# mgdesaix/WGSassign

Measured on AMD Instinct MI355X. Metric: EM SNP-updates/s (per-population update, n_call=100), higher is better.
Workload: dtype f64; 1 GPU; 1 GPU(s), SNP-sharded: synthetic Beagle 10000000 SNPs x 1000 ind, K=10, EM sweep; mode=exact, snps_per_gpu=10000000, gl_bytes_per_gpu=80000000000, comm_native_rccl=False, step=wgs_em_fit iteration (enqueued ahead of the host)

## Files before the change

wgsassign_amd/csrc/codes_kernels.hip:

```cpp
#include "common.h"

namespace {

typedef float f4 __attribute__((ext_vector_type(4)));
typedef const f4 __attribute__((address_space(1))) *gf4_ptr;
typedef uint32_t __attribute__((address_space(1))) *gu32_ptr;
typedef unsigned long long __attribute__((address_space(1))) *gu64_ptr;
typedef uint8_t __attribute__((address_space(1))) *gu8_ptr;

constexpr unsigned long long KEY_EMPTY = ~0ull;
constexpr int ENC_SLOTS = WGS_ENC_SLOTS;
constexpr int ENC_RMAX = 24;
constexpr int ENC_PD = ENC_SLOTS >= 2048 ? 2 : 1;
constexpr int ENC_UQ = ENC_SLOTS >= 2048 ? 4 : 2;

__device__ __forceinline__ unsigned hash32(unsigned g0, unsigned g1)
{
    const unsigned x = g0 ^ __builtin_rotateleft32(g1, 13);
    return __umul24(x, 0x9E3779u) ^ __builtin_rotateleft32(__umul24(x >> 8, 0x85EBCBu), 3);
}

struct EncodeArgs {
    float4 *const *base;
    const int32_t *npairs, *ncols;
    const SlabCodes *slabs;
    int32_t n_slabs;
    int64_t m, tiles;
    float2 *dict;
    uint8_t *ncls;
    int32_t drows, lrows;
    int32_t batch, batch_cap;
    int64_t unit_stride;
    uint8_t *sample;
    unsigned long long *stats;
    uint4 *wave_stats;
};

enum EncStat {
    ST_SUM_NCLS = 0,
    ST_RICH = 1,
    ST_CMAX = 2,
    ST_ROWS_BATCH = 3,
    ST_UNUSED = 4,
    ST_ROUNDS = 5,
    ST_BUFFERS = 6,
    ST_DIRECT = 7,
    ST_COUNT = 8
};

#ifdef WGS_ENC_STATS
__device__ unsigned long long g_enc_stats[8];
#define ENC_CLOCK(i) do { const unsigned long long now_ = clock64(); stat_[i] += now_ - mark_; mark_ = now_; } while (0)
#else
#define ENC_CLOCK(i) do { } while (0)
#endif

template <int SNPS, bool SAMPLE>
__global__ __launch_bounds__(64, ENC_SLOTS >= 2048 ? 2 : 4) void class_encode_kernel(EncodeArgs A)
{
#ifdef WGS_ENC_STATS
    unsigned long long stat_[4] = {0, 0, 0, 0}, mark_ = clock64();
#endif
    constexpr int COLS = 64 / SNPS, T = ENC_SLOTS / SNPS, NW = T / 64;
    constexpr unsigned TMASK = T - 1, HSHIFT = T == 64 ? 26 : (T == 128 ? 25 : 24);
    constexpr int NL = 4 * ENC_UQ;
    __shared__ unsigned long long keys[ENC_SLOTS];
    __shared__ __align__(16) uint8_t gid_of[ENC_SLOTS];
    __shared__ __align__(16) uint8_t slot_of[ENC_SLOTS];
    const int lane = threadIdx.x;
    const int s = lane & (SNPS - 1), col = lane / SNPS;
    const int64_t unit = (int64_t)blockIdx.x * A.unit_stride;
    const int64_t tile = unit / (64 / SNPS);
    const int sub = (int)(unit - tile * (64 / SNPS));
    if (tile >= A.tiles) return;
    const int ls = sub * SNPS + s;
    const int64_t snp = tile * 64 + ls;

#pragma unroll
    for (int i = 0; i < ENC_SLOTS / 64; ++i) keys[i * 64 + lane] = KEY_EMPTY;
    __builtin_amdgcn_fence(__ATOMIC_RELEASE, "wavefront");

    bool rich = false;
    unsigned n_rounds = 0, n_buffers = 0;
    int nid = 0;

    auto snp_or = [&](bool v) {
        int x = v ? 1 : 0;
#pragma unroll
        for (int d = SNPS; d < 64; d <<= 1) x |= __shfl_xor(x, d, 64);
        return x != 0;
    };
    auto snp_or64 = [&](unsigned long long v) {
        unsigned lo = (unsigned)v, hi = (unsigned)(v >> 32);
#pragma unroll
        for (int d = SNPS; d < 64; d <<= 1) {
            lo |= (unsigned)__shfl_xor((int)lo, d, 64);
            hi |= (unsigned)__shfl_xor((int)hi, d, 64);
        }
        return ((unsigned long long)hi << 32) | lo;
    };
    auto snp_scan = [&](int cnt, int &pre, int &tot) {
        pre = 0;
        tot = 0;
#pragma unroll
        for (int c = 0; c < COLS; ++c) {
            const int v = __shfl(cnt, c * SNPS + s, 64);
            if (c < col) pre += v;
            tot += v;
        }
    };
    auto wave_max = [&](int v) {
#pragma unroll
        for (int off = 32; off > 0; off >>= 1) v = max(v, __shfl_xor(v, off, 64));
        return v;
    };
    auto probe = [&](unsigned slot, unsigned long long key) { return atomicCAS(&keys[slot * SNPS + s], KEY_EMPTY, key); };
    auto set_bit = [&](unsigned long long (&m)[NW], unsigned id) {
#pragma unroll
        for (int w = 0; w < NW; ++w)
            if (NW == 1 || (id >> 6) == (unsigned)w) m[w] |= 1ull << (id & 63u);
    };
    auto bits_below = [&](const unsigned long long (&m)[NW], unsigned id) {
        int r = 0;
#pragma unroll
        for (int w = 0; w < NW; ++w) {
            const unsigned long long below = (id >> 6) > (unsigned)w ? ~0ull : ((id >> 6) == (unsigned)w ? (1ull << (id & 63u)) - 1ull : 0ull);
            r += __popcll(m[w] & below);
        }
        return r;
    };
    auto count_bits = [&](const unsigned long long (&m)[NW]) {
        int r = 0;
#pragma unroll
        for (int w = 0; w < NW; ++w) r += __popcll(m[w]);
        return r;
    };
    auto pop_lowest = [&](unsigned long long (&m)[NW]) {
        int pos = 0;
        bool done = false;
#pragma unroll
        for (int w = 0; w < NW; ++w) {
            if (!done && m[w]) {
                pos = 64 * w + __builtin_ctzll(m[w]);
                m[w] &= m[w] - 1ull;
                done = true;
            }
        }
        return pos;
    };

    ENC_CLOCK(0);
    for (int g = 0; g < A.n_slabs; ++g) {
        const int np = A.npairs[g], nc = A.ncols[g];
        const SlabCodes sc = A.slabs[g];
        const int nquads = sc.nquads;
        if (nquads == 0) continue;
        gf4_ptr src = (gf4_ptr)A.base[g] + tile * np * 64 + ls;
        gu32_ptr cw = (gu32_ptr)sc.codes + tile * nquads * 64 + ls;
        unsigned long long seen[NW];
#pragma unroll
        for (int w = 0; w < NW; ++w) seen[w] = 0ull;
        f4 nxt[ENC_PD][ENC_UQ][2];
        auto fetch = [&](int qb, f4 (&dst)[ENC_UQ][2]) {
#pragma unroll
            for (int u = 0; u < ENC_UQ; ++u) {
                const int q = qb + u * COLS + col;
                dst[u][0] = __builtin_nontemporal_load(src + (int64_t)min(2 * q, np - 1) * 64);
                dst[u][1] = __builtin_nontemporal_load(src + (int64_t)min(2 * q + 1, np - 1) * 64);
            }
        };
        constexpr int QSTEP = COLS * ENC_UQ;
#pragma unroll
        for (int d = 0; d < ENC_PD; ++d)
            if (d == 0 || d * QSTEP < nquads) fetch(d * QSTEP, nxt[d]);
        for (int qb = 0; qb < nquads; qb += QSTEP) {
            f4 v[ENC_UQ][2];
#pragma unroll
            for (int u = 0; u < ENC_UQ; ++u) v[u][0] = nxt[0][u][0], v[u][1] = nxt[0][u][1];
#pragma unroll
            for (int d = 0; d + 1 < ENC_PD; ++d)
#pragma unroll
                for (int u = 0; u < ENC_UQ; ++u) nxt[d][u][0] = nxt[d + 1][u][0], nxt[d][u][1] = nxt[d + 1][u][1];
            if (qb + ENC_PD * QSTEP < nquads) fetch(qb + ENC_PD * QSTEP, nxt[ENC_PD - 1]);
            unsigned long long key[NL], old[NL];
            unsigned slot[NL];
#pragma unroll
            for (int u = 0; u < ENC_UQ; ++u) {
#pragma unroll
                for (int h = 0; h < 4; ++h) {
                    const f4 vv = v[u][h >> 1];
                    const unsigned g0 = __float_as_uint((h & 1) ? vv.z : vv.x), g1 = __float_as_uint((h & 1) ? vv.w : vv.y);
                    key[4 * u + h] = ((unsigned long long)g1 << 32) | g0;
                    slot[4 * u + h] = hash32(g0, g1) >> HSHIFT;
                }
            }
            bool pend[NL], live[NL];
            const bool plain = 4 * (qb + COLS * ENC_UQ) <= nc && !__any(rich);
            if (plain) {
#pragma unroll
                for (int i = 0; i < NL; ++i) old[i] = probe(slot[i], key[i]);
#pragma unroll
                for (int i = 0; i < NL; ++i) {
                    live[i] = true;
                    pend[i] = old[i] != KEY_EMPTY && old[i] != key[i];
                }
            } else {
#pragma unroll
                for (int u = 0; u < ENC_UQ; ++u) {
                    const int q = qb + u * COLS + col;
#pragma unroll
                    for (int h = 0; h < 4; ++h) {
                        const int i = 4 * u + h;
                        live[i] = 4 * q + h < nc && !rich;
                        old[i] = key[i];
                        if (live[i]) old[i] = probe(slot[i], key[i]);
                    }
                }
#pragma unroll
                for (int i = 0; i < NL; ++i) pend[i] = live[i] && old[i] != KEY_EMPTY && old[i] != key[i];
            }
            bool any_pend = false;
#pragma unroll
            for (int i = 0; i < NL; ++i) any_pend = any_pend || pend[i];
            int rounds = 0;
            while (__any(any_pend)) {
                if (++rounds > ENC_RMAX) {
                    rich = rich || any_pend;
                    break;
                }
#pragma unroll
                for (int i = 0; i < NL; ++i) {
                    if (__any(pend[i])) {
                        if (pend[i]) {
                            slot[i] = (slot[i] + 1) & TMASK;
                            old[i] = probe(slot[i], key[i]);
                        }
                    }
                }
                any_pend = false;
#pragma unroll
                for (int i = 0; i < NL; ++i) {
                    pend[i] = pend[i] && old[i] != KEY_EMPTY && old[i] != key[i];
                    any_pend = any_pend || pend[i];
                }
            }
            n_rounds += (unsigned)rounds;
            ++n_buffers;
            int ins = 0;
#pragma unroll
            for (int i = 0; i < NL; ++i) ins += (live[i] && !pend[i] && old[i] == KEY_EMPTY) ? 1 : 0;
            if (__any(ins != 0)) {
                int pre, tot;
                snp_scan(ins, pre, tot);
                int id = nid + pre;
#pragma unroll
                for (int i = 0; i < NL; ++i) {
                    if (live[i] && !pend[i] && old[i] == KEY_EMPTY) {
                        gid_of[slot[i] * SNPS + s] = (uint8_t)min(id, 255);
                        if (id < T) slot_of[id * SNPS + s] = (uint8_t)slot[i];
                        ++id;
                    }
                }
                nid += tot;
                __builtin_amdgcn_fence(__ATOMIC_ACQ_REL, "wavefront");
            }
            unsigned cid[NL];
#pragma unroll
            for (int i = 0; i < NL; ++i) cid[i] = gid_of[slot[i] * SNPS + s];
            if (!plain) {
#pragma unroll
                for (int i = 0; i < NL; ++i) cid[i] = (live[i] && !pend[i]) ? cid[i] : 0u;
            }
#pragma unroll
            for (int i = 0; i < NL; ++i)
                if (plain || (live[i] && !pend[i])) set_bit(seen, cid[i] < (unsigned)T ? cid[i] : 0u);
            if (!SAMPLE) {
#pragma unroll
                for (int u = 0; u < ENC_UQ; ++u) {
                    const int q = qb + u * COLS + col;
                    if (plain || q < nquads) cw[(int64_t)q * 64] = cid[4 * u] | (cid[4 * u + 1] << 8) | (cid[4 * u + 2] << 16) | (cid[4 * u + 3] << 24);
                }
            }
        }
        ENC_CLOCK(1);
        if (nid > T || nid > 254) rich = true;
        rich = snp_or(rich);
#pragma unroll
        for (int w = 0; w < NW; ++w) seen[w] = snp_or64(seen[w]);
        const int nloc = count_bits(seen);
        if (SAMPLE) {
            if (col == 0) A.sample[((int64_t)blockIdx.x * (A.n_slabs + 1) + g) * SNPS + s] = (uint8_t)(snp < A.m ? (rich ? 255 : min(nloc, 254)) : 0);
        } else {
            const int wmax = wave_max(rich ? 255 : nloc);
            if (lane < SNPS / WGS_ENC_MIN_SNPS) ((gu8_ptr)sc.tile_rows)[tile * WGS_TILE_ROWS_BYTES + sub * (SNPS / WGS_ENC_MIN_SNPS) + lane] = (uint8_t)wmax;
            if (A.lrows > 0 && wmax <= A.lrows) {
                const int rows_w = wmax;
                gu64_ptr ld = (gu64_ptr)sc.ldict + (tile * A.lrows) * 64 + ls;
                unsigned long long walk[NW];
#pragma unroll
                for (int w = 0; w < NW; ++w) walk[w] = seen[w];
                for (int c = 0; c < col; ++c) (void)pop_lowest(walk);
                for (int r0 = col; r0 < rows_w; r0 += COLS) {
                    unsigned long long e = 0;
                    if (r0 < nloc) {
                        const int id = pop_lowest(walk);
                        e = keys[(unsigned)slot_of[id * SNPS + s] * SNPS + s];
                        for (int c = 1; c < COLS; ++c) (void)pop_lowest(walk);
                    }
                    ld[(int64_t)r0 * 64] = e;
                }
                gu32_ptr lw = (gu32_ptr)sc.lcodes + tile * nquads * 64 + ls;
                constexpr int PF = 8;
                for (int q0 = col; q0 < nquads; q0 += COLS * PF) {
                    uint32_t w[PF];
#pragma unroll
                    for (int u = 0; u < PF; ++u) w[u] = cw[(int64_t)min(q0 + u * COLS, nquads - 1) * 64];
#pragma unroll
                    for (int u = 0; u < PF; ++u) {
                        if (q0 + u * COLS < nquads) {
                            uint32_t o = 0;
#pragma unroll
                            for (int h = 0; h < 4; ++h) o |= (uint32_t)(bits_below(seen, (w[u] >> (8 * h)) & 255u) & 255) << (8 * h);
                            lw[(int64_t)(q0 + u * COLS) * 64] = o;
                        }
                    }
                }
            }
        }
    }

    __builtin_amdgcn_fence(__ATOMIC_ACQ_REL, "wavefront");
    ENC_CLOCK(2);
    const int ncls = nid;
    if (ncls > A.drows || ncls > 254 || ncls > T) rich = true;
    for (int r0 = col; r0 < min(ncls, T); r0 += COLS)
        if (keys[(unsigned)slot_of[r0 * SNPS + s] * SNPS + s] == KEY_EMPTY) rich = true;
    rich = snp_or(rich);
    if (SAMPLE) {
        if (col == 0) A.sample[((int64_t)blockIdx.x * (A.n_slabs + 1) + A.n_slabs) * SNPS + s] = (uint8_t)(snp < A.m ? (rich ? 255 : min(ncls, 254)) : 0);
        return;
    }
    int eff = rich ? 0 : ncls;
    auto group_sum = [&](int v) {
#pragma unroll
        for (int off = 1; off < 16; off <<= 1)
            if (off < A.batch && off < SNPS) v += __shfl_xor(v, off, 64);
        return v;
    };
    for (int it = 0; it < 16; ++it) {
        const int sum = group_sum(eff);
        if (!__any(sum > A.batch_cap)) break;
        int best = (eff << 8) | (63 - (lane & 15));
#pragma unroll
        for (int off = 1; off < 16; off <<= 1)
            if (off < A.batch && off < SNPS) best = max(best, __shfl_xor(best, off, 64));
        if (sum > A.batch_cap && (best & 255) == 63 - (lane & 15)) {
            eff = 0;
            rich = true;
        }
    }
    if (col == 0) ((gu8_ptr)A.ncls)[snp] = (uint8_t)eff;
    {
        const int mb = wave_max(group_sum(eff)), mc = wave_max(eff);
        unsigned long long tot = (unsigned long long)((col == 0 && snp < A.m) ? eff : 0), nrich = (col == 0 && snp < A.m && rich) ? 1ull : 0ull;
#pragma unroll
        for (int off = 32; off > 0; off >>= 1) {
            tot += __shfl_xor(tot, off, 64);
            nrich += __shfl_xor(nrich, off, 64);
        }
        if (lane == 0) {
            typedef unsigned u4 __attribute__((ext_vector_type(4)));
            typedef u4 __attribute__((address_space(1))) *gu4_ptr;
            gu4_ptr rec = (gu4_ptr)A.wave_stats + 2 * (int64_t)blockIdx.x;
            rec[0] = u4{(unsigned)tot, (unsigned)nrich, (unsigned)mc, (unsigned)mb};
            rec[1] = u4{n_rounds, n_buffers, 0u, 0u};
        }
    }
    const int wmax = min(wave_max(eff), A.drows);
    gu64_ptr dd = (gu64_ptr)A.dict + (tile * A.drows) * 64 + ls;
    for (int r0 = col; r0 < wmax; r0 += COLS)
        if (r0 < eff) dd[(int64_t)r0 * 64] = keys[(unsigned)slot_of[r0 * SNPS + s] * SNPS + s];
#ifdef WGS_ENC_STATS
    ENC_CLOCK(3);
    if (lane == 0 && (blockIdx.x & 63u) == 0u) {
#pragma unroll
        for (int i = 0; i < 4; ++i) atomicAdd(&g_enc_stats[i], stat_[i]);
        atomicAdd(&g_enc_stats[4], 1ull);
    }
#endif
}

__global__ __launch_bounds__(256) void sample_hist_kernel(const uint8_t *sample, int64_t units, int n_slabs, const int32_t *ncols, unsigned long long *hist)
{
    __shared__ unsigned int hg[256], hl[256];
    hg[threadIdx.x] = hl[threadIdx.x] = 0;
    __syncthreads();
    constexpr int W = WGS_ENC_MIN_SNPS;
    for (int64_t i = threadIdx.x; i < units * W; i += 256) {
        const uint8_t *row = sample + (i / W) * (n_slabs + 1) * W;
        const int x = (int)(i % W);
        const unsigned g = row[n_slabs * W + x];
        if (g == 0) continue;
        atomicAdd(&hg[g], 1u);
        for (int sl = 0; sl < n_slabs; ++sl)
            if (ncols[sl]) atomicAdd(&hl[row[sl * W + x]], 1u);
    }
    __syncthreads();
    hist[threadIdx.x] = hg[threadIdx.x];
    hist[256 + threadIdx.x] = hl[threadIdx.x];
}

__global__ __launch_bounds__(256) void encode_stats_kernel(const uint4 *wave_stats, int64_t units, const SlabCodes *slabs, int n_slabs, int64_t tiles,
                                                           unsigned lrows, unsigned long long *out)
{
    unsigned long long sum = 0, rich = 0, rounds = 0, buffers = 0, direct = 0;
    unsigned cmax = 0, rows = 0;
    const int64_t step = (int64_t)gridDim.x * 256;
    for (int64_t u = (int64_t)blockIdx.x * 256 + threadIdx.x; u < units; u += step) {
        const uint4 a = wave_stats[2 * u], b = wave_stats[2 * u + 1];
        sum += a.x, rich += a.y, cmax = max(cmax, a.z), rows = max(rows, a.w), rounds += b.x, buffers += b.y;
    }
    for (int g = 0; g < n_slabs; ++g) {
        if (slabs[g].nquads == 0) continue;
        const unsigned long long *tr = reinterpret_cast<const unsigned long long *>(slabs[g].tile_rows);
        for (int64_t t = (int64_t)blockIdx.x * 256 + threadIdx.x; t < tiles; t += step) {
            unsigned mx = 0;
#pragma unroll
            for (int x = 0; x < WGS_TILE_ROWS_BYTES / 8; ++x) {
                const unsigned long long w = tr[t * (WGS_TILE_ROWS_BYTES / 8) + x];
#pragma unroll
                for (int k = 0; k < 8; ++k) mx = max(mx, (unsigned)((w >> (8 * k)) & 255u));
            }
            direct += mx > lrows ? 1u : 0u;
        }
    }
#pragma unroll
    for (int off = 32; off > 0; off >>= 1) {
        sum += __shfl_xor(sum, off, 64), rich += __shfl_xor(rich, off, 64), rounds += __shfl_xor(rounds, off, 64);
        buffers += __shfl_xor(buffers, off, 64), direct += __shfl_xor(direct, off, 64);
        cmax = max(cmax, (unsigned)__shfl_xor((int)cmax, off, 64)), rows = max(rows, (unsigned)__shfl_xor((int)rows, off, 64));
    }
    if ((threadIdx.x & 63) == 0) {
        atomicAdd(out + ST_SUM_NCLS, sum);
        atomicAdd(out + ST_RICH, rich);
        atomicMax(out + ST_CMAX, (unsigned long long)cmax);
        atomicMax(out + ST_ROWS_BATCH, (unsigned long long)rows);
        atomicAdd(out + ST_ROUNDS, rounds);
        atomicAdd(out + ST_BUFFERS, buffers);
        atomicAdd(out + ST_DIRECT, direct);
    }
}

}

static EncodeArgs encode_args(wgs_beagle *b, wgs_codes *c, const int32_t *d_ncols, unsigned long long *d_stats)
{
    EncodeArgs A;
    A.base = b->d_base;
    A.npairs = b->d_npairs;
    A.ncols = d_ncols;
    A.slabs = c->d_slabs;
    A.n_slabs = b->n_groups;
    A.m = b->m;
    A.tiles = wgs_ntiles(b->m);
    A.dict = c->dict;
    A.ncls = c->ncls;
    A.drows = c->drows;
    A.lrows = c->lrows;
    A.batch = c->score_batch;
    A.batch_cap = WGS_BATCH_ROWS_CAP;
    A.unit_stride = 1;
    A.sample = nullptr;
    A.stats = d_stats;
    A.wave_stats = nullptr;
    return A;
}

static int encode_scratch(wgs_beagle *b, int32_t **d_ncols, unsigned long long **d_stats, size_t extra = 0)
{
    std::vector<int32_t> ncols(b->n_groups);
    for (int g = 0; g < b->n_groups; ++g) ncols[g] = b->slabs[g].ncols;
    void *ws = nullptr;
    const size_t stat_bytes = sizeof(unsigned long long) * ST_COUNT;
    if (wgs_ctx_workspace(b->ctx, stat_bytes + sizeof(int32_t) * (b->n_groups + 64) + extra, &ws)) return 1;
    *d_stats = reinterpret_cast<unsigned long long *>(ws);
    *d_ncols = reinterpret_cast<int32_t *>(reinterpret_cast<char *>(ws) + stat_bytes);
    HIP_TRY(hipMemsetAsync(*d_stats, 0, stat_bytes, b->ctx->stream));
    HIP_TRY(hipMemcpyAsync(*d_ncols, ncols.data(), sizeof(int32_t) * b->n_groups, hipMemcpyHostToDevice, b->ctx->stream));
    HIP_TRY(hipStreamSynchronize(b->ctx->stream));
    return 0;
}

int launch_class_sample(wgs_beagle *b, wgs_codes *c, int max_units, unsigned long long *hist_g, unsigned long long *hist_l, double *rounds_per_buffer)
{
    int32_t *d_ncols = nullptr;
    unsigned long long *d_stats = nullptr;
    const int64_t units = wgs_ntiles(b->m) * WGS_TILE_ROWS_BYTES;
    const int64_t stride = std::max<int64_t>(1, units / std::max(1, max_units));
    const int64_t grid = (units + stride - 1) / stride;
    const size_t sample_bytes = ((size_t)grid * (b->n_groups + 1) * WGS_ENC_MIN_SNPS + 7) / 8 * 8, hist_bytes = 512 * sizeof(unsigned long long);
    if (encode_scratch(b, &d_ncols, &d_stats, sample_bytes + hist_bytes + 8)) return 1;
    EncodeArgs A = encode_args(b, c, d_ncols, d_stats);
    A.drows = 254;
    A.lrows = 0;
    A.unit_stride = stride;
    A.sample = reinterpret_cast<uint8_t *>(d_ncols + b->n_groups + 64);
    unsigned long long *d_hist = reinterpret_cast<unsigned long long *>((reinterpret_cast<uintptr_t>(A.sample + sample_bytes) + 7) & ~(uintptr_t)7);
    hipLaunchKernelGGL((class_encode_kernel<WGS_ENC_MIN_SNPS, true>), dim3((unsigned)grid), dim3(64), 0, b->ctx->stream, A);
    HIP_TRY(hipGetLastError());
    hipLaunchKernelGGL(sample_hist_kernel, dim3(1), dim3(256), 0, b->ctx->stream, A.sample, grid, (int)b->n_groups, d_ncols, d_hist);
    HIP_TRY(hipGetLastError());
    unsigned long long *h = reinterpret_cast<unsigned long long *>(b->ctx->pinned);
    HIP_TRY(hipMemcpyAsync(h, d_hist, hist_bytes, hipMemcpyDeviceToHost, b->ctx->stream));
    HIP_TRY(hipStreamSynchronize(b->ctx->stream));
    for (int i = 0; i < 256; ++i) {
        hist_g[i] = h[i];
        hist_l[i] = h[256 + i];
    }
    if (rounds_per_buffer) *rounds_per_buffer = 0.0;
    return 0;
}

int launch_class_encode(wgs_beagle *b, wgs_codes *c)
{
    int32_t *d_ncols = nullptr;
    unsigned long long *d_stats = nullptr;
    if (encode_scratch(b, &d_ncols, &d_stats)) return 1;
    const int64_t tiles = wgs_ntiles(b->m);
    EncodeArgs A = encode_args(b, c, d_ncols, d_stats);
    const int64_t units = tiles * (64 / c->snps_per_wave);
    A.wave_stats = c->wave_stats;
    WGS_REQUIRE(units < (1ll << 31), "class encoder: %lld work units exceed one launch", (long long)units);
    HIP_TRY(hipEventRecord(b->ctx->enc_ev0, b->ctx->stream));
    if (c->snps_per_wave == WGS_ENC_SLOTS / 64) hipLaunchKernelGGL((class_encode_kernel<WGS_ENC_SLOTS / 64, false>), dim3((unsigned)units), dim3(64), 0, b->ctx->stream, A);
    else if (c->snps_per_wave == WGS_ENC_SLOTS / 128) hipLaunchKernelGGL((class_encode_kernel<WGS_ENC_SLOTS / 128, false>), dim3((unsigned)units), dim3(64), 0, b->ctx->stream, A);
    else hipLaunchKernelGGL((class_encode_kernel<WGS_ENC_SLOTS / 256, false>), dim3((unsigned)units), dim3(64), 0, b->ctx->stream, A);
    HIP_TRY(hipGetLastError());
    HIP_TRY(hipEventRecord(b->ctx->enc_ev1, b->ctx->stream));
    {
        const unsigned gx = (unsigned)std::max<int64_t>(1, std::min<int64_t>(512, (units + 255) / 256));
        hipLaunchKernelGGL(encode_stats_kernel, dim3(gx), dim3(256), 0, b->ctx->stream, c->wave_stats, units, c->d_slabs, (int)b->n_groups, tiles,
                           (unsigned)(c->lrows > 0 ? c->lrows : 255), d_stats);
        HIP_TRY(hipGetLastError());
    }
    unsigned long long *h = reinterpret_cast<unsigned long long *>(b->ctx->pinned);
    HIP_TRY(hipMemcpyAsync(h, d_stats, sizeof(unsigned long long) * 8, hipMemcpyDeviceToHost, b->ctx->stream));
    HIP_TRY(hipStreamSynchronize(b->ctx->stream));
#ifdef WGS_ENC_STATS
    {
        unsigned long long st[8] = {0}, zero[8] = {0};
        (void)hipMemcpyFromSymbol(st, HIP_SYMBOL(g_enc_stats), sizeof st);
        (void)hipMemcpyToSymbol(HIP_SYMBOL(g_enc_stats), zero, sizeof zero);
        const double w = st[4] ? (double)st[4] : 1.0;
        fprintf(stderr, "[encode stats] %llu wavefronts sampled; cycles per wavefront: before the slabs %.0f, the slabs' walks %.0f, the slabs' ends %.0f, the end %.0f\n",
                st[4], st[0] / w, st[1] / w, st[2] / w, st[3] / w);
    }
#endif
    float ev_ms = 0.0f;
    if (hipEventElapsedTime(&ev_ms, b->ctx->enc_ev0, b->ctx->enc_ev1) == hipSuccess) c->kernel_ms = ev_ms;
    c->sum_ncls = (double)h[ST_SUM_NCLS];
    c->rich_snps = (int64_t)h[ST_RICH];
    c->cmax = (int32_t)h[ST_CMAX];
    c->rows_batch = std::max<int32_t>(c->score_batch, (int32_t)h[ST_ROWS_BATCH]);
    c->probe_rounds = h[ST_BUFFERS] ? (double)h[ST_ROUNDS] / (double)h[ST_BUFFERS] : 0.0;
    int64_t slab_tiles = 0;
    for (int g = 0; g < b->n_groups; ++g) slab_tiles += c->slabs[g].nquads ? tiles : 0;
    c->local_direct_share = c->lrows > 0 && slab_tiles ? (double)h[ST_DIRECT] / (double)slab_tiles : 1.0;
    return 0;
}
```

Measured before the change: 7.728 billion SNP-updates/s.

## Restructure class encoder probe loop with ballots, 32-bit addressing and identity-code shortcut

Restructures the class-encode kernel's hash-probe inner loop into a templated walk_buffer. It specialises on plain versus tail buffers, with a half-width variant for short tails, uses wave ballots to track pending probes, and precomputes flat LDS indices. Global loads and stores move to 32-bit byte offsets from per-tile bases. A fast path skips the local-code remapping when local ids equal global ids. The intent is to cut ALU, addressing and branching cost in the one-time encoder, but the measured metric is EM-iteration throughput, which this kernel likely does not affect. It also adds an ncols limit check and a debug dump path.

```diff
diff --git a/wgsassign_amd/csrc/codes_kernels.hip b/wgsassign_amd/csrc/codes_kernels.hip
--- a/wgsassign_amd/csrc/codes_kernels.hip
+++ b/wgsassign_amd/csrc/codes_kernels.hip
@@ -1,3 +1,5 @@
+#include <type_traits>
+
 #include "common.h"
 
 namespace {
@@ -17,7 +19,9 @@
 __device__ __forceinline__ unsigned hash32(unsigned g0, unsigned g1)
 {
     const unsigned x = g0 ^ __builtin_rotateleft32(g1, 13);
-    return __umul24(x, 0x9E3779u) ^ __builtin_rotateleft32(__umul24(x >> 8, 0x85EBCBu), 3);
+    unsigned y;
+    asm("v_mul_u32_u24 %0, %1, %2" : "=v"(y) : "s"(0x85EBCBu), "v"(x >> 8));
+    return __umul24(x, 0x9E3779u) ^ __builtin_rotateleft32(y, 3);
 }
 
 struct EncodeArgs {
@@ -62,8 +66,7 @@
     unsigned long long stat_[4] = {0, 0, 0, 0}, mark_ = clock64();
 #endif
     constexpr int COLS = 64 / SNPS, T = ENC_SLOTS / SNPS, NW = T / 64;
-    constexpr unsigned TMASK = T - 1, HSHIFT = T == 64 ? 26 : (T == 128 ? 25 : 24);
-    constexpr int NL = 4 * ENC_UQ;
+    constexpr unsigned HSHIFT = T == 64 ? 26 : (T == 128 ? 25 : 24);
     __shared__ unsigned long long keys[ENC_SLOTS];
     __shared__ __align__(16) uint8_t gid_of[ENC_SLOTS];
     __shared__ __align__(16) uint8_t slot_of[ENC_SLOTS];
@@ -74,7 +77,6 @@
     const int sub = (int)(unit - tile * (64 / SNPS));
     if (tile >= A.tiles) return;
     const int ls = sub * SNPS + s;
-    const int64_t snp = tile * 64 + ls;
 
 #pragma unroll
     for (int i = 0; i < ENC_SLOTS / 64; ++i) keys[i * 64 + lane] = KEY_EMPTY;
@@ -114,11 +116,11 @@
         for (int off = 32; off > 0; off >>= 1) v = max(v, __shfl_xor(v, off, 64));
         return v;
     };
-    auto probe = [&](unsigned slot, unsigned long long key) { return atomicCAS(&keys[slot * SNPS + s], KEY_EMPTY, key); };
-    auto set_bit = [&](unsigned long long (&m)[NW], unsigned id) {
-#pragma unroll
-        for (int w = 0; w < NW; ++w)
-            if (NW == 1 || (id >> 6) == (unsigned)w) m[w] |= 1ull << (id & 63u);
+    auto probe = [&](unsigned at, unsigned long long key) { return atomicCAS(&keys[at], KEY_EMPTY, key); };
+    auto set_bit = [&](unsigned long long (&m)[NW], unsigned id, bool on) {
+        const unsigned long long bit = 1ull << (id & 63u);
+#pragma unroll
+        for (int w = 0; w < NW; ++w) m[w] |= (on & (NW == 1 || (id >> 6) == (unsigned)w)) ? bit : 0ull;
     };
     auto bits_below = [&](const unsigned long long (&m)[NW], unsigned id) {
         int r = 0;
@@ -147,6 +149,113 @@
             }
         }
         return pos;
+    };
+
+    auto walk_buffer = [&](auto plain_c, auto nu_c, const int qb, const f4 (&v)[ENC_UQ][2], const int nc, const int nquads, const uint32_t cw_at,
+                           gu8_ptr cw_tile, unsigned long long (&seen)[NW]) {
+        constexpr bool PLAIN = decltype(plain_c)::value;
+        constexpr int NU = decltype(nu_c)::value, NLB = 4 * NU;
+        unsigned long long key[NLB], old[NLB];
+        unsigned ki[NLB];
+        bool live[NLB];
+#pragma unroll
+        for (int u = 0; u < NU; ++u) {
+#pragma unroll
+            for (int h = 0; h < 4; ++h) {
+                const f4 vv = v[u][h >> 1];
+                const unsigned g0 = __float_as_uint((h & 1) ? vv.z : vv.x), g1 = __float_as_uint((h & 1) ? vv.w : vv.y);
+                key[4 * u + h] = ((unsigned long long)g1 << 32) | g0;
+                ki[4 * u + h] = (hash32(g0, g1) >> HSHIFT) * SNPS + s;
+                live[4 * u + h] = PLAIN || (4 * (qb + u * COLS + col) + h < nc && !rich);
+            }
+        }
+#pragma unroll
+        for (int i = 0; i < NLB; ++i) {
+            if (PLAIN) {
+                old[i] = probe(ki[i], key[i]);
+            } else {
+                old[i] = key[i];
+                if (live[i]) old[i] = probe(ki[i], key[i]);
+            }
+        }
+        unsigned long long pm[NLB], any_pend = 0ull, any_ins = 0ull;
+        auto pending = [&](int i) { return (old[i] != KEY_EMPTY) & (old[i] != key[i]); };
+        auto inserted = [&](int i) { return live[i] & (old[i] == KEY_EMPTY); };
+#pragma unroll
+        for (int i = 0; i < NLB; ++i) {
+            pm[i] = __builtin_amdgcn_ballot_w64(pending(i));
+            any_pend |= pm[i];
+            any_ins |= __builtin_amdgcn_ballot_w64(inserted(i));
+        }
+        int rounds = 0;
+        while (any_pend) {
+            if (++rounds > ENC_RMAX) {
+                bool p = false;
+#pragma unroll
+                for (int i = 0; i < NLB; ++i) p = p | pending(i);
+                rich = rich || p;
+                break;
+            }
+#pragma unroll
+            for (int i = 0; i < NLB; ++i) {
+                if (pm[i]) {
+                    if (pending(i)) {
+                        ki[i] = (ki[i] + SNPS) & (unsigned)(ENC_SLOTS - 1);
+                        old[i] = probe(ki[i], key[i]);
+                    }
+                }
+            }
+            any_pend = 0ull;
+#pragma unroll
+            for (int i = 0; i < NLB; ++i) {
+                if (pm[i]) {
+                    pm[i] = __builtin_amdgcn_ballot_w64(pending(i));
+                    any_ins |= __builtin_amdgcn_ballot_w64(inserted(i));
+                }
+                any_pend |= pm[i];
+            }
+        }
+        n_rounds += (unsigned)rounds;
+        ++n_buffers;
+        if (any_ins) {
+            int ins = 0;
+#pragma unroll
+            for (int i = 0; i < NLB; ++i) ins += inserted(i) ? 1 : 0;
+            if (__any(ins != 0)) {
+                int pre, tot;
+                snp_scan(ins, pre, tot);
+                int id = nid + pre;
+#pragma unroll
+                for (int i = 0; i < NLB; ++i) {
+                    if (inserted(i)) {
+                        gid_of[ki[i]] = (uint8_t)min(id, 255);
+                        if (id < T) slot_of[id * SNPS + s] = (uint8_t)(ki[i] / SNPS);
+                        ++id;
+                    }
+                }
+                nid += tot;
+                __builtin_amdgcn_fence(__ATOMIC_ACQ_REL, "wavefront");
+            }
+        }
+        unsigned cid[NLB];
+#pragma unroll
+        for (int i = 0; i < NLB; ++i) cid[i] = gid_of[ki[i]];
+#pragma unroll
+        for (int i = 0; i < NLB; ++i) {
+            bool ok = true;
+            if (!PLAIN) {
+                ok = live[i] & !pending(i);
+                cid[i] = ok ? cid[i] : 0u;
+            }
+            set_bit(seen, cid[i], ok);
+        }
+        if (!SAMPLE) {
+#pragma unroll
+            for (int u = 0; u < NU; ++u) {
+                const uint32_t word = cid[4 * u] | (cid[4 * u + 1] << 8) | (cid[4 * u + 2] << 16) | (cid[4 * u + 3] << 24);
+                if (PLAIN || qb + u * COLS + col < nquads) *(gu32_ptr)(cw_tile + (cw_at + (uint32_t)(u * COLS * 256))) = word;
+            }
+        }
     };
 
     ENC_CLOCK(0);
@@ -155,21 +264,38 @@
         const SlabCodes sc = A.slabs[g];
         const int nquads = sc.nquads;
         if (nquads == 0) continue;
-        gf4_ptr src = (gf4_ptr)A.base[g] + tile * np * 64 + ls;
-        gu32_ptr cw = (gu32_ptr)sc.codes + tile * nquads * 64 + ls;
+        typedef const char __attribute__((address_space(1))) *gc8_ptr;
+        gc8_ptr src_tile = (gc8_ptr)((gf4_ptr)A.base[g] + tile * np * 64);
+        gu8_ptr cw_tile = (gu8_ptr)((gu32_ptr)sc.codes + tile * nquads * 64);
+        const uint32_t ls16 = (uint32_t)ls * 16u, ls4 = (uint32_t)ls * 4u;
         unsigned long long seen[NW];
 #pragma unroll
         for (int w = 0; w < NW; ++w) seen[w] = 0ull;
         f4 nxt[ENC_PD][ENC_UQ][2];
+#pragma unroll
+        for (int d = 0; d < ENC_PD; ++d)
+#pragma unroll
+            for (int u = 0; u < ENC_UQ; ++u) nxt[d][u][0] = nxt[d][u][1] = f4{0.0f, 0.0f, 0.0f, 0.0f};
+        constexpr int QSTEP = COLS * ENC_UQ;
         auto fetch = [&](int qb, f4 (&dst)[ENC_UQ][2]) {
-#pragma unroll
-            for (int u = 0; u < ENC_UQ; ++u) {
-                const int q = qb + u * COLS + col;
-                dst[u][0] = __builtin_nontemporal_load(src + (int64_t)min(2 * q, np - 1) * 64);
-                dst[u][1] = __builtin_nontemporal_load(src + (int64_t)min(2 * q + 1, np - 1) * 64);
+            if (2 * (qb + QSTEP) <= np) {
+                const uint32_t at = (uint32_t)(qb + col) * 2048u + ls16;
+#pragma unroll
+                for (int u = 0; u < ENC_UQ; ++u) {
+                    dst[u][0] = __builtin_nontemporal_load((gf4_ptr)(src_tile + (at + (uint32_t)(u * COLS * 2048))));
+                    dst[u][1] = __builtin_nontemporal_load((gf4_ptr)(src_tile + (at + (uint32_t)(u * COLS * 2048 + 1024))));
+                }
+            } else {
+#pragma unroll
+                for (int u = 0; u < ENC_UQ; ++u) {
+                    if (qb + u * COLS < nquads) {
+                        const int q = qb + u * COLS + col;
+                        dst[u][0] = __builtin_nontemporal_load((gf4_ptr)(src_tile + ((uint32_t)min(2 * q, np - 1) * 1024u + ls16)));
+                        dst[u][1] = __builtin_nontemporal_load((gf4_ptr)(src_tile + ((uint32_t)min(2 * q + 1, np - 1) * 1024u + ls16)));
+                    }
+                }
             }
         };
-        constexpr int QSTEP = COLS * ENC_UQ;
 #pragma unroll
         for (int d = 0; d < ENC_PD; ++d)
             if (d == 0 || d * QSTEP < nquads) fetch(d * QSTEP, nxt[d]);
@@ -182,105 +308,11 @@
 #pragma unroll
                 for (int u = 0; u < ENC_UQ; ++u) nxt[d][u][0] = nxt[d + 1][u][0], nxt[d][u][1] = nxt[d + 1][u][1];
             if (qb + ENC_PD * QSTEP < nquads) fetch(qb + ENC_PD * QSTEP, nxt[ENC_PD - 1]);
-            unsigned long long key[NL], old[NL];
-            unsigned slot[NL];
-#pragma unroll
-            for (int u = 0; u < ENC_UQ; ++u) {
-#pragma unroll
-                for (int h = 0; h < 4; ++h) {
-                    const f4 vv = v[u][h >> 1];
-                    const unsigned g0 = __float_as_uint((h & 1) ? vv.z : vv.x), g1 = __float_as_uint((h & 1) ? vv.w : vv.y);
-                    key[4 * u + h] = ((unsigned long long)g1 << 32) | g0;
-                    slot[4 * u + h] = hash32(g0, g1) >> HSHIFT;
-                }
-            }
-            bool pend[NL], live[NL];
-            const bool plain = 4 * (qb + COLS * ENC_UQ) <= nc && !__any(rich);
-            if (plain) {
-#pragma unroll
-                for (int i = 0; i < NL; ++i) old[i] = probe(slot[i], key[i]);
-#pragma unroll
-                for (int i = 0; i < NL; ++i) {
-                    live[i] = true;
-                    pend[i] = old[i] != KEY_EMPTY && old[i] != key[i];
-                }
-            } else {
-#pragma unroll
-                for (int u = 0; u < ENC_UQ; ++u) {
-                    const int q = qb + u * COLS + col;
-#pragma unroll
-                    for (int h = 0; h < 4; ++h) {
-                        const int i = 4 * u + h;
-                        live[i] = 4 * q + h < nc && !rich;
-                        old[i] = key[i];
-                        if (live[i]) old[i] = probe(slot[i], key[i]);
-                    }
-                }
-#pragma unroll
-                for (int i = 0; i < NL; ++i) pend[i] = live[i] && old[i] != KEY_EMPTY && old[i] != key[i];
-            }
-            bool any_pend = false;
-#pragma unroll
-            for (int i = 0; i < NL; ++i) any_pend = any_pend || pend[i];
-            int rounds = 0;
-            while (__any(any_pend)) {
-                if (++rounds > ENC_RMAX) {
-                    rich = rich || any_pend;
-                    break;
-                }
-#pragma unroll
-                for (int i = 0; i < NL; ++i) {
-                    if (__any(pend[i])) {
-                        if (pend[i]) {
-                            slot[i] = (slot[i] + 1) & TMASK;
-                            old[i] = probe(slot[i], key[i]);
-                        }
-                    }
-                }
-                any_pend = false;
-#pragma unroll
-                for (int i = 0; i < NL; ++i) {
-                    pend[i] = pend[i] && old[i] != KEY_EMPTY && old[i] != key[i];
-                    any_pend = any_pend || pend[i];
-                }
-            }
-            n_rounds += (unsigned)rounds;
-            ++n_buffers;
-            int ins = 0;
-#pragma unroll
-            for (int i = 0; i < NL; ++i) ins += (live[i] && !pend[i] && old[i] == KEY_EMPTY) ? 1 : 0;
-            if (__any(ins != 0)) {
-                int pre, tot;
-                snp_scan(ins, pre, tot);
-                int id = nid + pre;
-#pragma unroll
-                for (int i = 0; i < NL; ++i) {
-                    if (live[i] && !pend[i] && old[i] == KEY_EMPTY) {
-                        gid_of[slot[i] * SNPS + s] = (uint8_t)min(id, 255);
-                        if (id < T) slot_of[id * SNPS + s] = (uint8_t)slot[i];
-                        ++id;
-                    }
-                }
-                nid += tot;
-                __builtin_amdgcn_fence(__ATOMIC_ACQ_REL, "wavefront");
-            }
-            unsigned cid[NL];
-#pragma unroll
-            for (int i = 0; i < NL; ++i) cid[i] = gid_of[slot[i] * SNPS + s];
-            if (!plain) {
-#pragma unroll
-                for (int i = 0; i < NL; ++i) cid[i] = (live[i] && !pend[i]) ? cid[i] : 0u;
-            }
-#pragma unroll
-            for (int i = 0; i < NL; ++i)
-                if (plain || (live[i] && !pend[i])) set_bit(seen, cid[i] < (unsigned)T ? cid[i] : 0u);
-            if (!SAMPLE) {
-#pragma unroll
-                for (int u = 0; u < ENC_UQ; ++u) {
-                    const int q = qb + u * COLS + col;
-                    if (plain || q < nquads) cw[(int64_t)q * 64] = cid[4 * u] | (cid[4 * u + 1] << 8) | (cid[4 * u + 2] << 16) | (cid[4 * u + 3] << 24);
-                }
-            }
+            const uint32_t cw_at = (uint32_t)(qb + col) * 256u + ls4;
+            const bool plain = 4 * (qb + QSTEP) <= nc && !__any(rich);
+            if (plain) walk_buffer(std::true_type(), std::integral_constant<int, ENC_UQ>(), qb, v, nc, nquads, cw_at, cw_tile, seen);
+            else if (qb + (ENC_UQ / 2) * COLS >= nquads) walk_buffer(std::false_type(), std::integral_constant<int, ENC_UQ / 2>(), qb, v, nc, nquads, cw_at, cw_tile, seen);
+            else walk_buffer(std::false_type(), std::integral_constant<int, ENC_UQ>(), qb, v, nc, nquads, cw_at, cw_tile, seen);
         }
         ENC_CLOCK(1);
         if (nid > T || nid > 254) rich = true;
@@ -289,39 +321,49 @@
         for (int w = 0; w < NW; ++w) seen[w] = snp_or64(seen[w]);
         const int nloc = count_bits(seen);
         if (SAMPLE) {
-            if (col == 0) A.sample[((int64_t)blockIdx.x * (A.n_slabs + 1) + g) * SNPS + s] = (uint8_t)(snp < A.m ? (rich ? 255 : min(nloc, 254)) : 0);
+            if (col == 0) A.sample[((int64_t)blockIdx.x * (A.n_slabs + 1) + g) * SNPS + s] = (uint8_t)(tile * 64 + ls < A.m ? (rich ? 255 : min(nloc, 254)) : 0);
         } else {
             const int wmax = wave_max(rich ? 255 : nloc);
             if (lane < SNPS / WGS_ENC_MIN_SNPS) ((gu8_ptr)sc.tile_rows)[tile * WGS_TILE_ROWS_BYTES + sub * (SNPS / WGS_ENC_MIN_SNPS) + lane] = (uint8_t)wmax;
             if (A.lrows > 0 && wmax <= A.lrows) {
                 const int rows_w = wmax;
-                gu64_ptr ld = (gu64_ptr)sc.ldict + (tile * A.lrows) * 64 + ls;
+                const bool same_numbers = __all(bits_below(seen, (unsigned)nloc) == nloc);
+                gu8_ptr ld_tile = (gu8_ptr)((gu64_ptr)sc.ldict + (tile * A.lrows) * 64);
+                const uint32_t ls8 = (uint32_t)ls * 8u;
                 unsigned long long walk[NW];
 #pragma unroll
                 for (int w = 0; w < NW; ++w) walk[w] = seen[w];
-                for (int c = 0; c < col; ++c) (void)pop_lowest(walk);
+                if (!same_numbers)
+                    for (int c = 0; c < col; ++c) (void)pop_lowest(walk);
                 for (int r0 = col; r0 < rows_w; r0 += COLS) {
                     unsigned long long e = 0;
                     if (r0 < nloc) {
-                        const int id = pop_lowest(walk);
+                        int id = r0;
+                        if (!same_numbers) {
+                            id = pop_lowest(walk);
+                            for (int c = 1; c < COLS; ++c) (void)pop_lowest(walk);
+                        }
                         e = keys[(unsigned)slot_of[id * SNPS + s] * SNPS + s];
-                        for (int c = 1; c < COLS; ++c) (void)pop_lowest(walk);
                     }
-                    ld[(int64_t)r0 * 64] = e;
+                    *(gu64_ptr)(ld_tile + ((uint32_t)r0 * 512u + ls8)) = e;
                 }
-                gu32_ptr lw = (gu32_ptr)sc.lcodes + tile * nquads * 64 + ls;
-                constexpr int PF = 8;
-                for (int q0 = col; q0 < nquads; q0 += COLS * PF) {
+                gu8_ptr lw_tile = (gu8_ptr)((gu32_ptr)sc.lcodes + tile * nquads * 64);
+                constexpr int PF = COLS >= 16 ? 2 : 4;
+                for (int q0 = 0; q0 < nquads; q0 += COLS * PF) {
                     uint32_t w[PF];
 #pragma unroll
-                    for (int u = 0; u < PF; ++u) w[u] = cw[(int64_t)min(q0 + u * COLS, nquads - 1) * 64];
+                    for (int u = 0; u < PF; ++u)
+                        if (q0 + u * COLS < nquads) w[u] = *(gu32_ptr)(cw_tile + ((uint32_t)min(q0 + u * COLS + col, nquads - 1) * 256u + ls4));
 #pragma unroll
                     for (int u = 0; u < PF; ++u) {
                         if (q0 + u * COLS < nquads) {
-                            uint32_t o = 0;
-#pragma unroll
-                            for (int h = 0; h < 4; ++h) o |= (uint32_t)(bits_below(seen, (w[u] >> (8 * h)) & 255u) & 255) << (8 * h);
-                            lw[(int64_t)(q0 + u * COLS) * 64] = o;
+                            uint32_t o = w[u];
+                            if (!same_numbers) {
+                                o = 0;
+#pragma unroll
+                                for (int h = 0; h < 4; ++h) o |= (uint32_t)(bits_below(seen, (w[u] >> (8 * h)) & 255u) & 255) << (8 * h);
+                            }
+                            if (q0 + u * COLS + col < nquads) *(gu32_ptr)(lw_tile + ((uint32_t)(q0 + u * COLS + col) * 256u + ls4)) = o;
                         }
                     }
                 }
@@ -331,6 +373,7 @@
 
     __builtin_amdgcn_fence(__ATOMIC_ACQ_REL, "wavefront");
     ENC_CLOCK(2);
+    const int64_t snp = tile * 64 + ls;
     const int ncls = nid;
     if (ncls > A.drows || ncls > 254 || ncls > T) rich = true;
     for (int r0 = col; r0 < min(ncls, T); r0 += COLS)
@@ -531,6 +574,14 @@
     const int64_t units = tiles * (64 / c->snps_per_wave);
     A.wave_stats = c->wave_stats;
     WGS_REQUIRE(units < (1ll << 31), "class encoder: %lld work units exceed one launch", (long long)units);
+    for (int g = 0; g < b->n_groups; ++g)
+        WGS_REQUIRE((int64_t)b->slabs[g].ncols < (1ll << 22), "class encoder: a slab of %lld individuals exceeds its addressing", (long long)b->slabs[g].ncols);
+#ifdef WGS_ENC_DUMP
+    {
+        const size_t head = ((sizeof(SlabCodes) * b->n_groups + 255) / 256) * 256;
+        if (b->pool_bytes > head) HIP_TRY(hipMemsetAsync(reinterpret_cast<char *>(b->pool) + head, 0, b->pool_bytes - head, b->ctx->stream));
+    }
+#endif
     HIP_TRY(hipEventRecord(b->ctx->enc_ev0, b->ctx->stream));
     if (c->snps_per_wave == WGS_ENC_SLOTS / 64) hipLaunchKernelGGL((class_encode_kernel<WGS_ENC_SLOTS / 64, false>), dim3((unsigned)units), dim3(64), 0, b->ctx->stream, A);
     else if (c->snps_per_wave == WGS_ENC_SLOTS / 128) hipLaunchKernelGGL((class_encode_kernel<WGS_ENC_SLOTS / 128, false>), dim3((unsigned)units), dim3(64), 0, b->ctx->stream, A);
@@ -546,6 +597,36 @@
     unsigned long long *h = reinterpret_cast<unsigned long long *>(b->ctx->pinned);
     HIP_TRY(hipMemcpyAsync(h, d_stats, sizeof(unsigned long long) * 8, hipMemcpyDeviceToHost, b->ctx->stream));
     HIP_TRY(hipStreamSynchronize(b->ctx->stream));
+#ifdef WGS_ENC_DUMP
+    {
+        auto digest = [&](const char *name, int g, const void *dev, size_t bytes) {
+            std::vector<unsigned long long> host((bytes + 7) / 8, 0ull);
+            if (bytes && hipMemcpy(host.data(), dev, bytes, hipMemcpyDeviceToHost) != hipSuccess) return;
+            unsigned long long a = 0x9E3779B97F4A7C15ull, x = 0ull;
+            for (size_t i = 0; i < host.size(); ++i) {
+                a = (a ^ host[i]) * 0x100000001B3ull;
+                a ^= a >> 29;
+                x += host[i] * (2 * (unsigned long long)i + 1);
+            }
+            fprintf(stderr, "[encode dump] %s[%d] %zu bytes %016llx %016llx\n", name, g, bytes, a, x);
+        };
+        digest("ncls", 0, c->ncls, (size_t)tiles * 64);
+        digest("dict", 0, c->dict, (size_t)tiles * c->drows * 64 * sizeof(float2));
+        digest("wave_stats", 0, c->wave_stats, sizeof(uint4) * 2 * (size_t)units);
+        digest("stats", 0, d_stats, sizeof(unsigned long long) * ST_COUNT);
+        for (int g = 0; g < b->n_groups; ++g) {
+            const SlabCodes &sl = c->slabs[g];
+            if (sl.nquads == 0) continue;
+            const size_t words = (size_t)tiles * sl.nquads * 64;
+            digest("codes", g, sl.codes, words * sizeof(uint32_t));
+            digest("tile_rows", g, sl.tile_rows, WGS_TILE_ROWS_BYTES * (size_t)tiles);
+            if (c->lrows > 0) {
+                digest("lcodes", g, sl.lcodes, words * sizeof(uint32_t));
+                digest("ldict", g, sl.ldict, (size_t)tiles * c->lrows * 64 * sizeof(float2));
+            }
+        }
+    }
+#endif
 #ifdef WGS_ENC_STATS
     {
         unsigned long long st[8] = {0}, zero[8] = {0};
```

Measured after the change: 7.521 billion SNP-updates/s. -2.7%, worse.
